# tjiiv-cprg/EPro-PnP

Hardware: AMD Instinct MI355X
Metric: PnP instances/sec (fwd+bwd, N=512 pts, 512 samples) (higher is better)
Workload: dtype f32; 1 GPU; C2 batched synthetic: 4096 objects/GPU x N=512 points, S=512 MC samples, K=4 AMIS iters, L=3 LM iters, EProPnP6DoF fwd+bwd; objects_per_gpu=4096, objects_total=4096, num_points=512, mc_samples=512, amis_iters=4, lm_iters=3, dof=6, parallelism=objects sharded x1, no data-path collective

## Files before the change

### epro-pnp_amd/csrc/amis_common.h

```cpp
#pragma once
#include "pnp_host.h"
#include "tuning.h"

namespace pnp {

typedef PNP_FIT_T fit_t;

__device__ __forceinline__ float sat_mul(float x, float one_v) {
  return __builtin_amdgcn_fmed3f(x * one_v, 0.0f, 1.0f);
}

__device__ __forceinline__ float sat_fma(float a, float b, float c) {
  return __builtin_amdgcn_fmed3f(fmaf(a, b, c), 0.0f, 1.0f);
}

__device__ __forceinline__ float clamp_below(float x, float lo) {
  int xi, li;
  memcpy(&xi, &x, 4);
  memcpy(&li, &lo, 4);
  const int mi = max(xi, li);
  float r;
  memcpy(&r, &mi, 4);
  return r;
}
// ... 8 lines not shown
  return h;
}

constexpr int kPropStride = 40;
constexpr int kVmTries = PNP_VM_TRIES;
constexpr int kRedStride = 68;
constexpr int kWaveRed = 16 * kRedStride + 64;

struct AmisParams {
  int S, K;
  int WP;
  float eps;
  int mle_iter;
  float dispersion;
  unsigned long long seed, offset;
  const unsigned long long* offset_dev;
  unsigned long long* advance;
  int* advance_ticket;
  int advance_count;
  int ablate;
  unsigned split_timeout;
  const float* dn_offset;
  float* dn_samples;
  float* dn_pose_opt;
  float* sample_costs;
};

template <int DOF>
PNP_FN void denormalise_pose_opt(const AmisParams& a, const float* __restrict__ pose_opt, int b) {
  constexpr int PL = PoseLen<DOF>::value;
  if (a.dn_offset == nullptr || a.dn_pose_opt == nullptr) return;
  float ps[PL], R[9];
#pragma unroll
  for (int i = 0; i < PL; ++i) ps[i] = pose_opt[(size_t)b * PL + i];
  pose_to_rot<DOF>(ps, R);
  shift_translation(ps, R, a.dn_offset[(size_t)b * 3], a.dn_offset[(size_t)b * 3 + 1], a.dn_offset[(size_t)b * 3 + 2], -1.0f);
#pragma unroll
  for (int i = 0; i < PL; ++i) a.dn_pose_opt[(size_t)b * PL + i] = ps[i];
}

__device__ __forceinline__ void advance_counters(const AmisParams& a, int expected) {
  if (a.advance == nullptr) return;
  if (threadIdx.x == 0) {
    if (atomicAdd(a.advance_ticket, 1) == expected - 1) {
      for (int i = 0; i < a.advance_count; ++i) atomicAdd(&a.advance[i], 1ull);
      atomicExch(a.advance_ticket, 0);
    }
  }
}


__device__ __forceinline__ constexpr int tri(int i, int j) { return i * (i + 1) / 2 + j; }


PNP_FIT_FN void fit_translation(fit_t (&C)[3][3], const float* fallback_diag, float* rec) {
  fit_t invd[3];
  const bool ok = cholesky<3, fit_t>(C, invd);
  rec[37] = ok ? 0.f : 1.f;
  if (!ok) {
#pragma unroll
    for (int i = 0; i < 3; ++i) {
#pragma unroll
      for (int j = 0; j < 3; ++j) C[i][j] = (i == j) ? (fit_t)fallback_diag[i] : fit_t(0);
      invd[i] = fit_t(1) / (fit_t)fallback_diag[i];
    }
  }
  fit_t Li[3][3];
  tri_inverse<3, fit_t>(C, invd, Li);
  float sl = 0.f;
#pragma unroll
  for (int i = 0; i < 3; ++i) {
    sl += fast_log((float)C[i][i]);
#pragma unroll
    for (int j = 0; j <= i; ++j) {
      rec[3 + tri(i, j)] = (float)C[i][j];
      rec[9 + tri(i, j)] = (float)Li[i][j];
    }
  }
  rec[15] = student_t3_log_norm(sl);
}

constexpr int kRefitMaxVals = 21;
constexpr int kRefitRedFloats = kRefitMaxVals * kSumTRow + 24;

template <int NV>
PNP_FN void wave_sum_t(float (&v)[NV], float* lds, int lane) {
  static_assert(NV <= kRefitMaxVals, "scratch rows");
  float* tot = lds + kRefitMaxVals * kSumTRow;
#pragma unroll
  for (int i = 0; i < NV; ++i) lds[i * kSumTRow + lane] = v[i];
  wave_lds_fence();
#pragma unroll
  for (int base = 0; base < NV; base += 16) {
    const int row = base + (lane >> 2);
    float part = 0.f;
    if (row < NV) {
      const float4* r = reinterpret_cast<const float4*>(lds + row * kSumTRow + 16 * (lane & 3));
      const float4 a = r[0], b = r[1], c = r[2], d = r[3];
      part = (((a.x + a.y) + (a.z + a.w)) + ((b.x + b.y) + (b.z + b.w))) + (((c.x + c.y) + (c.z + c.w)) + ((d.x + d.y) + (d.z + d.w)));
    }
    part = quad_sum(part);
    if (row < NV && (lane & 3) == 0) tot[row] = part;
  }
  wave_lds_fence();
#pragma unroll
  for (int i = 0; i < NV; ++i) v[i] = tot[i];
  wave_lds_fence();
}

template <int NV>
PNP_FN void refit_sum(float (&v)[NV], float* scratch, int lane) {
  if (scratch != nullptr) {
    wave_sum_t<NV>(v, scratch, lane);
  } else {
#pragma unroll
    for (int i = 0; i < NV; ++i) v[i] = wave_sum(v[i]);
  }
}

PNP_FIT_FN void fit_factor_pair(fit_t (&A)[4][4], int which, float dispersion, const float (&fallback)[4], float* rec) {
  const fit_t m01 = A[0][0] * A[1][1] - A[0][1] * A[1][0], m02 = A[0][0] * A[1][2] - A[0][2] * A[1][0],
               m03 = A[0][0] * A[1][3] - A[0][3] * A[1][0], m12 = A[0][1] * A[1][2] - A[0][2] * A[1][1],
               m13 = A[0][1] * A[1][3] - A[0][3] * A[1][1], m23 = A[0][2] * A[1][3] - A[0][3] * A[1][2];
  const fit_t n01 = A[2][0] * A[3][1] - A[2][1] * A[3][0], n02 = A[2][0] * A[3][2] - A[2][2] * A[3][0],
               n03 = A[2][0] * A[3][3] - A[2][3] * A[3][0], n12 = A[2][1] * A[3][2] - A[2][2] * A[3][1],
               n13 = A[2][1] * A[3][3] - A[2][3] * A[3][1], n23 = A[2][2] * A[3][3] - A[2][3] * A[3][2];
  const float det = (float)(m01 * n23 - m02 * n13 + m03 * n12 + m12 * n03 - m13 * n02 + m23 * n01);
  const fit_t add = (which == 0) ? (fit_t)(sqrtf(sqrtf(det)) * dispersion) : fit_t(0);
  fit_t invd[4];
#pragma unroll
  for (int i = 0; i < 4; ++i) A[i][i] += add;
  const bool ok = cholesky<4, fit_t>(A, invd) && (add == add);
  if (!ok) {
#pragma unroll
    for (int i = 0; i < 4; ++i) {
#pragma unroll
      for (int j = 0; j < 4; ++j) A[i][j] = (i == j) ? (fit_t)fallback[i] : fit_t(0);
      invd[i] = fit_t(1) / (fit_t)fallback[i];
    }
  }
  fit_t Li[4][4];
  tri_inverse<4, fit_t>(A, invd, Li);
  float sl = 0.f;
  const int oL = which ? 3 : 16, oLi = which ? 9 : 26;
#pragma unroll
  for (int i = 0; i < 4; ++i) {
    sl += fast_log((float)A[i][i]);
#pragma unroll
    for (int j = 0; j <= i; ++j) {
      if (which == 0 || i < 3) {
        rec[oL + tri(i, j)] = (float)A[i][j];
        rec[oLi + tri(i, j)] = (float)Li[i][j];
      }
    }
  }
  rec[which ? 15 : 36] = which ? student_t3_log_norm(sl) : sl;
  rec[which ? 37 : 38] = ok ? 0.f : 1.f;
}

template <int DOF>
PNP_FIT_FN void initial_fit(const float* pose_opt, const float* cov, float eps, float dispersion, float* rec, int which = 0) {
  if (which == 0) {
    rec[0] = pose_opt[0]; rec[1] = pose_opt[1]; rec[2] = pose_opt[2];
    rec[39] = 0.f;
  }
  if (DOF == 4) {
    rec[37] = rec[38] = 0.f;
    fit_t Ct[3][3];
#pragma unroll
    for (int i = 0; i < 3; ++i)
#pragma unroll
      for (int j = 0; j < 3; ++j) Ct[i][j] = (fit_t)cov[i * DOF + j];
    const float dflt[3] = {1.0f, 1.0f, 4.0f};
    fit_translation(Ct, dflt, rec);
    rec[16] = pose_opt[3];
    const float kappa = 0.33f / fmaxf(cov[3 * 4 + 3], eps);
    rec[17] = kappa;
    rec[18] = log_i0(kappa);
#pragma unroll
    for (int i = 19; i < 37; ++i) rec[i] = 0.f;
  } else {
    fit_t Cr[3][3], Ci[3][3];
#pragma unroll
    for (int i = 0; i < 3; ++i)
#pragma unroll
      for (int j = 0; j < 3; ++j) Cr[i][j] = (fit_t)cov[(3 + i) * 6 + 3 + j];
    fit_t invd4[4];
    {
      const fit_t c00 = Cr[1][1] * Cr[2][2] - Cr[1][2] * Cr[2][1], c01 = Cr[1][2] * Cr[2][0] - Cr[1][0] * Cr[2][2],
                   c02 = Cr[1][0] * Cr[2][1] - Cr[1][1] * Cr[2][0];
      const fit_t idet = fit_t(1) / (Cr[0][0] * c00 + Cr[0][1] * c01 + Cr[0][2] * c02);
      Ci[0][0] = c00 * idet; Ci[1][0] = c01 * idet; Ci[2][0] = c02 * idet;
      Ci[0][1] = (Cr[0][2] * Cr[2][1] - Cr[0][1] * Cr[2][2]) * idet;
      Ci[1][1] = (Cr[0][0] * Cr[2][2] - Cr[0][2] * Cr[2][0]) * idet;
      Ci[2][1] = (Cr[0][1] * Cr[2][0] - Cr[0][0] * Cr[2][1]) * idet;
      Ci[0][2] = (Cr[0][1] * Cr[1][2] - Cr[0][2] * Cr[1][1]) * idet;
// ... 249 lines not shown
        ps[3] = v0 * inr; ps[4] = v1 * inr; ps[5] = v2 * inr; ps[6] = v3 * inr;
      }
    } else {
      const int n_u = (int)rintf(0.25f * (float)s);
      auto uniforms = [&](int att, float& u1, float& u2, float& u3) {
        if (noise != nullptr) {
          const float* nz = noise + (((size_t)b * K + it) * s + n) * NZ + 4 + 3 * att;
          u1 = nz[0]; u2 = nz[1]; u3 = nz[2];
        } else {
          const Philox4 r = philox4x32_10((uint32_t)b, (uint32_t)m, (uint32_t)a.offset,
                                          (uint32_t)(a.offset >> 32) * 64u + 8u + (uint32_t)att, (uint32_t)a.seed,
                                          (uint32_t)(a.seed >> 32));
          u1 = (float)(r.v[0] >> 8) * (1.0f / 16777216.0f);
          u2 = (float)(r.v[1] >> 8) * (1.0f / 16777216.0f);
          u3 = (float)(r.v[2] >> 8) * (1.0f / 16777216.0f);
        }
      };
      if (n < n_u) {
        float u1, u2, u3;
        uniforms(0, u1, u2, u3);
        ps[3] = (u1 * 2.0f - 1.0f) * 3.14159265358979f;
      } else {
        ps[3] = vm_sample_bounded(rec[16], rec[17], uniforms);
      }
    }
    PNP_REFIT_ADD(3, rot_t0_);
#pragma unroll
    for (int i = 0; i < PL; ++i) smp[i * S + m] = ps[i];
    if (pose_samples != nullptr) store_pose<PL>(pose_samples + ((size_t)m * p.B + b) * PL, ps);
    {
      float R[9], KR[9], Kt[3];
      pose_to_rot<DOF>(ps, R);
      if (pose_samples != nullptr && a.dn_samples != nullptr) {
        float pd[PL];
#pragma unroll
        for (int i = 0; i < PL; ++i) pd[i] = ps[i];
        shift_translation(pd, R, a.dn_offset[(size_t)b * 3], a.dn_offset[(size_t)b * 3 + 1], a.dn_offset[(size_t)b * 3 + 2], -1.0f);
        store_pose<PL>(a.dn_samples + ((size_t)m * p.B + b) * PL, pd);
      }
      compose_kr_kt(Kc, R, ps, KR, Kt);
      float4* row = reinterpret_cast<float4*>(ptab + 12 * (n - n0));
      row[0] = make_float4(KR[0], KR[1], KR[2], Kt[0]);
      row[1] = make_float4(KR[3], KR[4], KR[5], Kt[1]);
      row[2] = make_float4(KR[6], KR[7], KR[8], Kt[2]);
    }
  }

}

template <int DOF>
PNP_FN void amis_weights(const AmisCtx& cx, const AmisParams& a, int it, int WP) {
  constexpr int PL = PoseLen<DOF>::value;
  float* smp = cx.smp; float* cst = cx.cst; float* mixl = cx.mixl; float* lgw = cx.lgw; float* cpart = cx.cpart; float* prop = cx.prop;
  const int S = cx.S, s = cx.s, T = cx.T, tid = cx.tid;
  const float* rec = prop + it * kPropStride;
  const int M = (it + 1) * s;
  const float log_n = logf((float)(it + 1));
  for (int m = tid; m < M; m += T) {
    float ps[PL];
#pragma unroll
    for (int i = 0; i < PL; ++i) ps[i] = smp[i * S + m];
    float mix;
    if (m >= it * s) {
      if (WP > 0) {
        float c = cpart[m - it * s];
        for (int q = 1; q < WP; ++q) c += cpart[q * cx.cstride + (m - it * s)];
        cst[m] = c;
      }
      if (PNP_ABLATED(a, 4)) {
        mix = 0.f;
      } else {
        mix = proposal_logprob<DOF>(prop, ps);
        for (int j = 1; j <= it; ++j) mix = log_add_exp(mix, proposal_logprob<DOF>(prop + j * kPropStride, ps));
      }
    } else {
      mix = PNP_ABLATED(a, 4) ? 0.f : log_add_exp(mixl[m], proposal_logprob<DOF>(rec, ps));
    }
    mixl[m] = mix;
    lgw[m] = -cst[m] - (mix - log_n);
  }

}

template <int DOF>
PNP_FN void amis_refit(const AmisCtx& cx, const AmisParams& a, int it) {
  float* smp = cx.smp; float* lgw = cx.lgw; float* prop = cx.prop; float* red = cx.red;
  const int S = cx.S, s = cx.s;
  const float* rec = prop + it * kPropStride;
  const int M = (it + 1) * s;
  float* nrec = prop + (it + 1) * kPropStride;
  if (wave_id() != 0) {
    amis_base_noise<DOF>(cx, a, it + 1, 64);
    __syncthreads();
    return;
  }
  const int T = 64, tid = cx.tid;
  PNP_REFIT_BEGIN();
  if (PNP_ABLATED(a, 2)) {
    for (int i = tid; i < kPropStride; i += T) nrec[i] = rec[i];
    __syncthreads();
    return;
  }
  float mx = -INFINITY;
  for (int m = tid; m < M; m += T) mx = fmaxf(mx, lgw[m]);
  mx = wave_max(mx);
  const float p0 = rec[0], p1 = rec[1], p2 = rec[2];
  if (DOF == 6) {
    float mom[21];
#pragma unroll
    for (int i = 0; i < 21; ++i) mom[i] = 0.f;
    if (PNP_ABLATED(a, 8)) mom[0] = mom[4] = mom[6] = mom[9] = mom[10] = mom[12] = mom[15] = mom[19] = mom[20] = 1.f;
    else
    for (int m = tid; m < M; m += T) {
      const float e = fast_exp(lgw[m] - mx);
      const float d0 = smp[m] - p0, d1 = smp[S + m] - p1, d2 = smp[2 * S + m] - p2;
      mom[0] += e;
      mom[1] += e * d0; mom[2] += e * d1; mom[3] += e * d2;
      mom[4] += e * d0 * d0; mom[5] += e * d1 * d0; mom[6] += e * d1 * d1;
      mom[7] += e * d2 * d0; mom[8] += e * d2 * d1; mom[9] += e * d2 * d2;
      const float q0 = smp[3 * S + m], q1 = smp[4 * S + m], q2 = smp[5 * S + m], q3 = smp[6 * S + m];
      const float iw = e * fast_rcp(fmaxf(q0 * q0 + q1 * q1 + q2 * q2 + q3 * q3, a.eps));
      mom[10] += iw * q0 * q0;
      mom[11] += iw * q1 * q0; mom[12] += iw * q1 * q1;
      mom[13] += iw * q2 * q0; mom[14] += iw * q2 * q1; mom[15] += iw * q2 * q2;
      mom[16] += iw * q3 * q0; mom[17] += iw * q3 * q1; mom[18] += iw * q3 * q2; mom[19] += iw * q3 * q3;
      mom[20] += iw;
    }
    if (!PNP_ABLATED(a, 16)) refit_sum<21>(mom, cx.rred, tid);
    const float invZ = 1.0f / mom[0];
    const float dl0 = mom[1] * invZ, dl1 = mom[2] * invZ, dl2 = mom[3] * invZ;
    const float mu0 = p0 + dl0, mu1 = p1 + dl1, mu2 = p2 + dl2;
    float c6[6];
    c6[0] = mom[4] * invZ - dl0 * dl0; c6[1] = mom[5] * invZ - dl1 * dl0; c6[2] = mom[6] * invZ - dl1 * dl1;
    c6[3] = mom[7] * invZ - dl2 * dl0; c6[4] = mom[8] * invZ - dl2 * dl1; c6[5] = mom[9] * invZ - dl2 * dl2;
    float acc[11];
#pragma unroll
    for (int i = 0; i < 11; ++i) acc[i] = mom[10 + i];
    PNP_REFIT_PHASE(0);
    float Lf[10], Ld[4];
    for (int r = 1; r < a.mle_iter; ++r) {
      if (tid == 0) {
        fit_t Sg[4][4], invd[4];
        const fit_t inorm = fit_t(1) / (fit_t)acc[10];
#pragma unroll
        for (int i = 0; i < 4; ++i)
#pragma unroll
          for (int j = 0; j <= i; ++j) {
            const fit_t v = (fit_t)acc[tri(i, j)] * inorm + ((i == j) ? (fit_t)a.eps : fit_t(0));
            Sg[i][j] = v;
            Sg[j][i] = v;
          }
        cholesky<4, fit_t>(Sg, invd);
#pragma unroll
        for (int i = 0; i < 4; ++i) {
          red[10 + i] = (float)invd[i];
#pragma unroll
          for (int j = 0; j < i; ++j) red[tri(i, j)] = (float)Sg[i][j];
        }
      }
      wave_lds_fence();
#pragma unroll
      for (int i = 0; i < 10; ++i) Lf[i] = red[i];
#pragma unroll
      for (int i = 0; i < 4; ++i) Ld[i] = red[10 + i];
      wave_lds_fence();
#pragma unroll
      for (int i = 0; i < 11; ++i) acc[i] = 0.f;
      for (int m = tid; m < M; m += T) {
        const float e = fast_exp(lgw[m] - mx);
        const float q0 = smp[3 * S + m], q1 = smp[4 * S + m], q2 = smp[5 * S + m], q3 = smp[6 * S + m];
        const float y0 = q0 * Ld[0];
        const float y1 = fmaf(-Lf[tri(1, 0)], y0, q1) * Ld[1];
        const float y2 = fmaf(-Lf[tri(2, 1)], y1, fmaf(-Lf[tri(2, 0)], y0, q2)) * Ld[2];
        const float y3 = fmaf(-Lf[tri(3, 2)], y2, fmaf(-Lf[tri(3, 1)], y1, fmaf(-Lf[tri(3, 0)], y0, q3))) * Ld[3];
        const float Mq = fmaf(y3, y3, fmaf(y2, y2, fmaf(y1, y1, y0 * y0)));
        const float iw = e * fast_rcp(fmaxf(Mq, a.eps));
        acc[10] += iw;
        acc[0] += iw * q0 * q0;
        acc[1] += iw * q1 * q0; acc[2] += iw * q1 * q1;
        acc[3] += iw * q2 * q0; acc[4] += iw * q2 * q1; acc[5] += iw * q2 * q2;
        acc[6] += iw * q3 * q0; acc[7] += iw * q3 * q1; acc[8] += iw * q3 * q2; acc[9] += iw * q3 * q3;
      }
      refit_sum<11>(acc, cx.rred, tid);
    }
    PNP_REFIT_PHASE(1);
    if (tid < 2) {
      if (tid == 0) {
        nrec[0] = mu0; nrec[1] = mu1; nrec[2] = mu2;
        nrec[39] = 0.f;
      }
      fit_t A4[4][4];
      const fit_t inorm = (a.mle_iter > 0) ? fit_t(1) / (fit_t)acc[10] : fit_t(0);
#pragma unroll
      for (int i = 0; i < 4; ++i)
#pragma unroll
        for (int j = 0; j <= i; ++j) {
          fit_t v = (a.mle_iter > 0) ? (fit_t)acc[tri(i, j)] * inorm + ((i == j) ? (fit_t)a.eps : fit_t(0))
                                      : ((i == j) ? fit_t(1) : fit_t(0));
          if (tid == 1) v = (i < 3) ? (fit_t)c6[tri(i, j)] : ((i == j) ? fit_t(1) : fit_t(0));
          A4[i][j] = v;
          A4[j][i] = v;
        }
      const float dflt[4] = {1.f, 1.f, 1.f, 1.f};
      fit_factor_pair(A4, tid, a.dispersion, dflt, nrec);
    }
    PNP_REFIT_PHASE(2);
  } else {
    float mom[12];
#pragma unroll
    for (int i = 0; i < 12; ++i) mom[i] = 0.f;
    for (int m = tid; m < M; m += T) {
      const float e = fast_exp(lgw[m] - mx);
      const float d0 = smp[m] - p0, d1 = smp[S + m] - p1, d2 = smp[2 * S + m] - p2;
      mom[0] += e;
      mom[1] += e * d0; mom[2] += e * d1; mom[3] += e * d2;
      mom[4] += e * d0 * d0; mom[5] += e * d1 * d0; mom[6] += e * d1 * d1;
      mom[7] += e * d2 * d0; mom[8] += e * d2 * d1; mom[9] += e * d2 * d2;
      const float yaw = smp[3 * S + m];
      float sy, cy;
      sincos_rad(yaw, sy, cy);
      mom[10] += e * sy;
      mom[11] += e * cy;
    }
    refit_sum<12>(mom, cx.rred, tid);
    const float invZ = 1.0f / mom[0];
    const float dl0 = mom[1] * invZ, dl1 = mom[2] * invZ, dl2 = mom[3] * invZ;
    const float mu0 = p0 + dl0, mu1 = p1 + dl1, mu2 = p2 + dl2;
    float c8[8];
    c8[0] = mom[4] * invZ - dl0 * dl0; c8[1] = mom[5] * invZ - dl1 * dl0; c8[2] = mom[6] * invZ - dl1 * dl1;
    c8[3] = mom[7] * invZ - dl2 * dl0; c8[4] = mom[8] * invZ - dl2 * dl1; c8[5] = mom[9] * invZ - dl2 * dl2;
    c8[6] = mom[10] * invZ;
    c8[7] = mom[11] * invZ;
    if (tid == 0) {
      nrec[0] = mu0; nrec[1] = mu1; nrec[2] = mu2;
      fit_t Ct[3][3];
#pragma unroll
      for (int i = 0; i < 3; ++i)
#pragma unroll
        for (int j = 0; j <= i; ++j) {
          Ct[i][j] = (fit_t)c8[tri(i, j)];
          Ct[j][i] = (fit_t)c8[tri(i, j)];
        }
      const float dflt[3] = {1.f, 1.f, 4.f};
      nrec[38] = nrec[39] = 0.f;
      fit_translation(Ct, dflt, nrec);
      nrec[16] = atan2f(c8[6], c8[7]);
      const float r_sq = c8[6] * c8[6] + c8[7] * c8[7];
      const float kappa = 0.33f * fmaxf(sqrtf(r_sq), a.eps) * (2.f - r_sq) / fmaxf(1.f - r_sq, a.eps);
      nrec[17] = kappa;
      nrec[18] = log_i0(kappa);
#pragma unroll
      for (int i = 19; i < 37; ++i) nrec[i] = 0.f;
    }
  }
  __syncthreads();
}

}
```

### epro-pnp_amd/csrc/amis_forward_mfma.hip

```cpp
#include "amis_common.h"
#include "dispatch.h"

namespace pnp {



template <bool BOUNDS, bool FOLDED = false>
__device__ __forceinline__ void huber_cost_4(const floatx4& hx, const floatx4& hy, const floatx4& hz, const float4& w4,
                                             float zmin_v, float one_v, const Bounds& bd, f32x2 (&acc2)[2]) {
  static_assert(!(BOUNDS && FOLDED), "the clamp acts on the un-weighted projection");
  const f32x2 wu2 = {w4.x, w4.x}, wv2 = {w4.y, w4.y}, cu2 = {w4.z, w4.z}, cv2 = {w4.w, w4.w};
  const f32x2 mhalf = {-0.5f, -0.5f};
#pragma unroll
  for (int h = 0; h < 2; ++h) {
    const float z0 = clamp_below(hz[2 * h], zmin_v), z1 = clamp_below(hz[2 * h + 1], zmin_v);
    const f32x2 rz2 = {fast_rcp(z0), fast_rcp(z1)};
    const f32x2 hx2 = {hx[2 * h], hx[2 * h + 1]}, hy2 = {hy[2 * h], hy[2 * h + 1]};
    f32x2 rx2, ry2;
    if (FOLDED) {
      rx2 = fma2(hx2, rz2, cu2);
      ry2 = fma2(hy2, rz2, cv2);
    } else {
      f32x2 px2 = hx2 * rz2, py2 = hy2 * rz2;
      if (BOUNDS) {
        px2 = f32x2{clamp_lu(px2[0], bd.lbx, bd.ubx), clamp_lu(px2[1], bd.lbx, bd.ubx)};
        py2 = f32x2{clamp_lu(py2[0], bd.lby, bd.uby), clamp_lu(py2[1], bd.lby, bd.uby)};
      }
      rx2 = fma2(px2, wu2, cu2);
      ry2 = fma2(py2, wv2, cv2);
    }
    const f32x2 s2 = fma2(rx2, rx2, ry2 * ry2);
    const f32x2 rho2 = {fast_sqrt(s2[0]), fast_sqrt(s2[1])};
    const f32x2 m2 = {sat_mul(rho2[0], one_v), sat_mul(rho2[1], one_v)};
    acc2[h] = fma2(m2, fma2(mhalf, m2, rho2), acc2[h]);
  }
}

constexpr int kChunk = 1024;

struct MfmaShape {
  int chunk;
  int s16;
  int ahead;
  int chunks;
};

template <int DOF, bool BOUNDS, int NPT, bool SPILL = false, bool SPLIT = false, bool BF16 = false, bool CHUNKED = false>
__global__ __launch_bounds__(512, SPLIT ? 2 : (DOF == 6 ? (NPT <= 8 ? (BF16 ? PNP_FWD_BF16_MINW : PNP_FWD_MINW) : 2) : (NPT <= 2 ? 3 : 2))) void amis_forward_mfma_kernel(Problem p, AmisParams a_in, MfmaShape sh,
                                                                  const float* __restrict__ pose_opt,
                                                                  const float* __restrict__ pose_cov,
                                                                  const float* __restrict__ noise,
                                                                  float* __restrict__ pose_samples,
                                                                  float* __restrict__ logweights,
                                                                  float* __restrict__ proposals,
                                                                  float* __restrict__ spill, int nsplit,
                                                                  float* __restrict__ xch) {
  static_assert(!SPILL || NPT == 0, "the spill variant streams the points");
  static_assert(!SPLIT || NPT > 0, "the split over workgroups is a register-mode variant");
  constexpr int PL = PoseLen<DOF>::value;
  const int G = SPLIT ? nsplit : 1;
  static_assert(!CHUNKED || (NPT > 0 && !SPLIT && !SPILL), "chunks are a register-mode variant of the one-workgroup kernel");
  const int CH = CHUNKED ? sh.chunks : 1;
  const int GT = SPLIT ? G : CH;
  int b, part = 0;
  if (SPLIT) {
    const int g = (int)blockIdx.x, per = (p.B + 7) >> 3, idx = g >> 3;
    part = idx % G;
    b = (g & 7) * per + idx / G;
  } else {
    b = object_of_block(p.B);
  }
  if (b >= p.B) return;
  AmisParams a = a_in;
  if (a.offset_dev != nullptr) a.offset += *a.offset_dev;
  const int T = (int)blockDim.x, tid = (int)threadIdx.x, lane = lane_id(), wv = wave_id(), W = T >> 6;
  const int S = a.S, K = a.K, s = S / K, s16 = sh.s16, NC = sh.chunk;

  PNP_PHASES_BEGIN(6);
  PNP_DYN_SMEM(float, smem);
  constexpr bool kRegs = NPT > 0;
  static_assert(!BF16 || NPT > 0, "the split projection is a register-mode variant");
  constexpr bool kBf = BF16;
  typedef ProjOp<kBf> Proj;
  constexpr bool kFold = kRegs && !BOUNDS && !kBf;
  const int WPs = kRegs ? (G > 1 ? G : W) : 1;
  const int cpart_rows = kRegs ? (SPLIT ? W + G : W) : 1;
  float* ptab = smem;
  float* pB = ptab + 12 * s16;
  float* pW = pB + 4 * NC;
  float* smp = SPILL ? spill + (size_t)b * (PL + 3) * S : pW + 4 * NC;
  float* cst = smp + PL * S;
  float* mixl = cst + S;
  float* lgw = mixl + S;
  float* cpart = SPILL ? pW + 4 * NC : smp + (((PL + 3) * S + 3) & ~3);
  float* gath = cpart + W * s16;
  float* prop = cpart + cpart_rows * s16 + (SPLIT ? 4 : 0);
  float* red = prop + K * kPropStride;
  float* rred = red + 256;
  float* nzb = (s <= T) ? ptab : rred + kRefitRedFloats;

  float Kc[9], delta;
  Bounds bd;
  load_camera<BOUNDS>(p, b, Kc, bd, delta);
  const float zmin_v = to_vgpr(p.z_min), one_v = to_vgpr(1.0f);
  const HuberScale hs = huber_scale(delta);
  const float inv_delta = hs.inv_delta, delta_sq = hs.delta_sq;

  const bool tiled = SPILL && s > s16;
  AmisCtx cx;
  cx.ptab = ptab; cx.smp = smp; cx.cst = cst; cx.mixl = mixl; cx.lgw = lgw; cx.cpart = SPLIT ? gath : cpart; cx.prop = prop; cx.red = red;
  cx.S = S; cx.K = K; cx.s = s; cx.T = T; cx.tid = tid; cx.b = b; cx.cstride = s16;
  cx.nzb = (noise == nullptr && W > 1 && sh.ahead) ? nzb : nullptr;
  cx.rred = rred;

  if (!tiled)
    for (int i = tid; i < 12 * (s16 - s); i += T) ptab[12 * s + i] = 0.f;
  if (tid < (DOF == 6 ? 2 : 1))
    initial_fit<DOF>(pose_opt + (size_t)b * PL, pose_cov + (size_t)b * DOF * DOF, a.eps, a.dispersion, prop, tid);
  if (part == 0 && tid == T - 1) denormalise_pose_opt<DOF>(a, pose_opt, b);
  const int nchunk = kRegs ? 1 : (p.N + NC - 1) / NC;
  auto load_chunk = [&](int c0) {
    const int cnt = min(NC, ((p.N - c0 + 15) >> 4) << 4);
    for (int n = tid; n < cnt; n += T) {
      const Point q = load_point(p, b, c0 + n);
      reinterpret_cast<float4*>(pB)[n] = make_float4(q.X, q.Y, q.Z, 1.0f);
      const float wu = q.wu * inv_delta, wv = q.wv * inv_delta;
      reinterpret_cast<float4*>(pW)[n] = make_float4(wu, wv, -q.u * wu, -q.v * wv);
    }
  };
  typename Proj::T rB[kRegs ? NPT : 1];
  float4 rW[kRegs ? NPT : 1];
  auto load_tiles = [&](int pt) {
#pragma unroll
    for (int i = 0; i < (kRegs ? NPT : 1); ++i) {
      const Point q = load_point(p, b, ((pt * W + wv) + GT * W * i) * 16 + (lane & 15));
      const int k4 = lane >> 4;
      const float bval = (k4 == 0) ? q.X : (k4 == 1) ? q.Y : (k4 == 2) ? q.Z : 1.0f;
      rB[i] = Proj::b(bval);
      const float wu = q.wu * inv_delta, wv = q.wv * inv_delta;
      rW[i] = kFold ? make_float4(bval * wu, bval * wv, -q.u * wu, -q.v * wv) : make_float4(wu, wv, -q.u * wu, -q.v * wv);
    }
  };
  if (kRegs) {
    if constexpr (!CHUNKED) load_tiles(part);
  } else if (nchunk == 1) {
    load_chunk(0);
  }
  amis_base_noise<DOF>(cx, a, 0, 64);
  __syncthreads();

  const int g4 = (lane >> 4) * 4, col = lane & 15, kk = lane >> 4;
  auto sweep_regs = [&](bool accumulate = false) {
    const floatx4 zero = {0.f, 0.f, 0.f, 0.f};
    for (int t = 0; t < (s16 >> 4); ++t) {
      const float* arow = ptab + 12 * (t * 16 + col) + kk;
      const typename Proj::T ax = Proj::a(arow[0]), ay = Proj::a(arow[4]), az = Proj::a(arow[8]);
      f32x2 acc2[2] = {f32x2{0.f, 0.f}, f32x2{0.f, 0.f}};
      constexpr int NT = kRegs ? NPT : 1;
      constexpr bool kPipe = (PNP_FWD_PIPE != 0) && !kFold && NT >= 4;
      floatx4 hxn = zero, hyn = zero, hzn = zero;
      if (kPipe) {
        hxn = Proj::mma(ax, rB[0], zero); hyn = Proj::mma(ay, rB[0], zero); hzn = Proj::mma(az, rB[0], zero);
      }
#pragma unroll
      for (int i = 0; i < NT; ++i) {
        floatx4 hx, hy, hz;
        if constexpr (kFold) {
          hx = mfma_16x16x4(ax, rW[i].x, zero);
          hy = mfma_16x16x4(ay, rW[i].y, zero);
          hz = mfma_16x16x4(az, rB[i], zero);
        } else if constexpr (kPipe) {
          hx = hxn; hy = hyn; hz = hzn;
          if (i + 1 < NT) {
            hxn = Proj::mma(ax, rB[i + 1], zero);
            hyn = Proj::mma(ay, rB[i + 1], zero);
            hzn = Proj::mma(az, rB[i + 1], zero);
            sched_fence();
          }
        } else {
          hx = Proj::mma(ax, rB[i], zero);
          hy = Proj::mma(ay, rB[i], zero);
          hz = Proj::mma(az, rB[i], zero);
        }
        huber_cost_4<BOUNDS, kFold>(hx, hy, hz, rW[i], zmin_v, one_v, bd, acc2);
      }
      const float acc[4] = {acc2[0][0], acc2[0][1], acc2[1][0], acc2[1][1]};
      const float tot = row_sum16_of4(acc);
      if (col < 4) {
        float* dst = cpart + wv * s16 + t * 16 + g4 + col;
        if constexpr (CHUNKED) *dst = accumulate ? fmaf(tot, delta_sq, *dst) : tot * delta_sq;
        else *dst = tot * delta_sq;
      }
    }
  };
  PNP_PHASE(0);
  unsigned gone_parts = 0u;
  for (int it = 0; it < K; ++it) {
    for (int n0 = 0; n0 < (SPILL ? s : 1); n0 += (SPILL ? s16 : 1)) {
    const int cnt = min(s16, s - n0), cnt16 = (cnt + 15) & ~15;
    if (tiled) {
      if (n0 > 0) __syncthreads();
      for (int i = tid; i < 12 * (cnt16 - cnt); i += T) ptab[12 * cnt + i] = 0.f;
    }
    if (!PNP_ABLATED(a, 32) || it == 0)
      amis_draw<DOF>(cx, p, a, it, Kc, noise, part == 0 ? pose_samples : nullptr, n0, tiled ? cnt : -1);
    __syncthreads();
    PNP_PHASE(1);

    if (PNP_ABLATED(a, 1)) {
      for (int n = tid; n < s; n += T) cpart[n] = 1.0f;
    } else if (kRegs) {
      if constexpr (!CHUNKED) {
        sweep_regs();
      } else {
        for (int c = 0; c < CH; ++c) {
          load_tiles(c);
          sweep_regs(c > 0);
        }
      }
    } else
    for (int ch = 0; ch < nchunk; ++ch) {
      const int c0 = ch * NC;
      if (nchunk > 1) {
        if (ch > 0 || it > 0) __syncthreads();
        load_chunk(c0);
        __syncthreads();
      }
      const int npt = (min(NC, p.N - c0) + 15) >> 4;
      for (int t = wv; t < (cnt16 >> 4); t += W) {
        const float* arow = ptab + 12 * (t * 16 + col) + kk;
        const float ax = arow[0], ay = arow[4], az = arow[8];
        f32x2 acc2[2] = {f32x2{0.f, 0.f}, f32x2{0.f, 0.f}};
        const floatx4 zero = {0.f, 0.f, 0.f, 0.f};
        float bq = pB[4 * col + kk];
        float4 w4 = reinterpret_cast<const float4*>(pW)[col];
        floatx4 hx = mfma_16x16x4(ax, bq, zero), hy = mfma_16x16x4(ay, bq, zero), hz = mfma_16x16x4(az, bq, zero);
        for (int q = 0; q < npt; ++q) {
          const int qn = min(q + 1, npt - 1);
          const float bn = pB[4 * (qn * 16 + col) + kk];
          const float4 wn = reinterpret_cast<const float4*>(pW)[qn * 16 + col];
          const floatx4 hxn = mfma_16x16x4(ax, bn, zero);
          const floatx4 hyn = mfma_16x16x4(ay, bn, zero);
          const floatx4 hzn = mfma_16x16x4(az, bn, zero);
          huber_cost_4<BOUNDS>(hx, hy, hz, w4, zmin_v, one_v, bd, acc2);
          hx = hxn; hy = hyn; hz = hzn; w4 = wn;
        }
        const float acc[4] = {acc2[0][0], acc2[0][1], acc2[1][0], acc2[1][1]};
        const float tot = row_sum16_of4(acc);
        if (col < 4) {
          const int pose = t * 16 + g4 + col;
          cpart[pose] = (ch == 0) ? tot * delta_sq : fmaf(tot, delta_sq, cpart[pose]);
        }
      }
    }
    __syncthreads();
    if (tiled)
      for (int m = tid; m < cnt; m += T) cst[it * s + n0 + m] = cpart[m];
    }
    if (kRegs && SPLIT) {
      unsigned* slot = reinterpret_cast<unsigned*>(xch) + (((size_t)b * K + it) * G) * s16;
      unsigned* missw = reinterpret_cast<unsigned*>(gath + G * s16);
      for (int m = tid; m < s; m += T) {
        float c = cpart[m];
        for (int w = 1; w < W; ++w) c += cpart[w * s16 + m];
        const unsigned bits = xwg_payload(c);
        xwg_store(slot + part * s16 + m, bits);
        gath[part * s16 + m] = bits_f32(bits);
      }
      if (tid == 0) *missw = 0u;
      __syncthreads();
      unsigned miss = 0u;
      for (int i = tid; i < G * s; i += T) {
        const int q = i / s, m = i - q * s;
        if (q == part) continue;
        const unsigned v = xwg_poll(slot + q * s16 + m, (((miss | gone_parts) >> q) & 1u) ? 0u : a.split_timeout);
        if (v == kXwgEmpty) miss |= 1u << q; else gath[q * s16 + m] = bits_f32(v);
      }
      if (miss) atomicOr(reinterpret_cast<int*>(missw), (int)miss);
      __syncthreads();
      unsigned todo = *missw;
      gone_parts |= todo;
      if (todo) {
        if (tid == 0) raise_status(p, EPROPNP_ST_SPLIT_TIMEOUT, b);
        for (int q = 0; q < G; ++q) {
          if (!((todo >> q) & 1u)) continue;
          load_tiles(q);
          sweep_regs();
          __syncthreads();
          for (int m = tid; m < s; m += T) {
            float c = cpart[m];
            for (int w = 1; w < W; ++w) c += cpart[w * s16 + m];
            gath[q * s16 + m] = bits_f32(xwg_payload(c));
          }
          __syncthreads();
        }
        load_tiles(part);
      }
    }
    PNP_PHASE(2);

    if (tiled) __syncthreads();
    AmisCtx cxw = cx;
    cxw.tid = (int)f32_bits(to_vgpr(bits_f32((unsigned)tid)));
    amis_weights<DOF>(cxw, a, it, tiled ? 0 : WPs);
    __syncthreads();
    PNP_PHASE(3);
    if (it == K - 1) break;
    amis_refit<DOF>(cxw, a, it);
    PNP_PHASE(4);
  }

  if (part == 0) {
    int st_bits = 0;
    for (int m = tid; m < S; m += T) {
      const float lw = lgw[m];
      logweights[(size_t)m * p.B + b] = lw;
      if (a.sample_costs != nullptr) a.sample_costs[(size_t)m * p.B + b] = cst[m];
      st_bits |= (lw == lw && lw != INFINITY) ? 0 : EPROPNP_ST_NONFINITE_WEIGHT;
    }
    for (int i = tid; i < K; i += T)
      st_bits |= (prop[i * kPropStride + 37] != 0.f || prop[i * kPropStride + 38] != 0.f) ? EPROPNP_ST_CHOL_FALLBACK : 0;
    raise_status(p, st_bits, b);
  }
  if (proposals != nullptr && part == 0)
    for (int i = tid; i < K * kPropStride; i += T) proposals[(size_t)b * K * kPropStride + i] = prop[i];
  PNP_PHASE(5);
  advance_counters(a, p.B * G);
  PNP_PHASES_FLUSH(6);
}

int tuning_phase_cycles(unsigned long long* out, int reset) { return tuning::read_cycles(out, reset, true); }

template <class F>
static int dispatch_npt(int npt, F&& f) {
  switch (npt) {
    case 0: return f(ic<0>{});
    case 1: return f(ic<1>{});
    case 2: return f(ic<2>{});
    case 4: return f(ic<4>{});
    case 8: return f(ic<8>{});
    case 12: return f(ic<12>{});
    default: return f(ic<16>{});
  }
}

static int forward_split_parts(int B, int ptiles) {
  const long wgs = padded_object_grid(B), cus = device_cu_count();
  int g = 8;
  while (g > 1 && (wgs * g > cus || 8 * g > ptiles)) g >>= 1;
  if (g < 4) g = 1;
  { int ov[1]; if (env_ints("EPROPNP_FWD_SPLIT", ov, 1) && (ov[0] == 1 || ov[0] == 2 || ov[0] == 4 || ov[0] == 8) && wgs * ov[0] <= 4096 && 4 * ov[0] <= ptiles) g = ov[0]; }
  return g;
}

unsigned long long amis_forward_split_bytes(const epropnp_problem* prob, int mc_samples, int num_iter) {
  if (prob == nullptr || prob->num_obj <= 0 || num_iter <= 0 || mc_samples % num_iter != 0) return 0;
  const int ptiles = (prob->num_pts + 15) / 16;
  const int g = forward_split_parts(prob->num_obj, ptiles);
  if (g <= 1 || (ptiles + 4 * g - 1) / (4 * g) > 8) return 0;
  const int s16 = ((mc_samples / num_iter + 15) / 16) * 16;
  return sizeof(float) * (unsigned long long)prob->num_obj * num_iter * g * s16;
}

struct FwdPlan {
  MfmaShape sh;
  int waves, npt, G;
  size_t smem;
  bool bf16, spilled, truncated, chunked;
};

static int plan_amis_forward(const epropnp_problem* prob, int S, int K, unsigned long long scratch_bytes, FwdPlan* out) {
  const int B = prob->num_obj, N = prob->num_pts;
  const int s = S / K;
  const int PL = prob->dof == 6 ? 7 : 4;
  MfmaShape& sh = out->sh;
  sh.s16 = ((s + 15) / 16) * 16;
  const int ptiles = (N + 15) / 16;
  const int npt_opts[6] = {1, 2, 4, 8, 12, 16};
  int waves = 4, npt = 0, best = 1 << 30;
  for (int w : {4, 8, 2, 1}) {
    for (int o : npt_opts) {
      if (w * o >= ptiles && w * o < best) { best = w * o; waves = w; npt = o; }
      if (w * o >= ptiles) break;
    }
  }
  if (prob->dof == 4 && npt >= 12) npt = 0;
  if (B < 512 && waves == 4 && npt == 8) { waves = 8; npt = 4; }
  { int ov[2]; if (tune_ints("fwd_mfma", ov, 2) && (ov[0] == 1 || ov[0] == 2 || ov[0] == 4 || ov[0] == 8) && (ov[1] == 0 || ov[1] == 1 || ov[1] == 2 || ov[1] == 4 || ov[1] == 8 || ov[1] == 12 || ov[1] == 16) && (ov[1] == 0 || ov[0] * ov[1] >= ptiles)) { waves = ov[0]; npt = ov[1]; } }
  if (npt == 0) {
    sh.chunk = ((N + 15) / 16) * 16;
    if (sh.chunk > kChunk) sh.chunk = kChunk;
    if (best == (1 << 30)) waves = 4;
    const int tiles = sh.s16 / 16;
    while (waves > 1 && waves > tiles) waves /= 2;
  } else {
    sh.chunk = 0;
  }
  int G = 1;
  {
    const int g = forward_split_parts(B, ptiles);
    const size_t need = sizeof(float) * (size_t)B * K * g * sh.s16;
    int ovf[1];
    const bool forced = env_ints("EPROPNP_FWD_SPLIT", ovf, 1);
    if (g > 1 && (forced || (scratch_bytes != 0 && scratch_bytes >= need))) {
      int per_wave = (ptiles + 4 * g - 1) / (4 * g), o = 1;
      while (o < per_wave) o *= 2;
      if (o <= 8) { G = g; waves = 4; npt = o; sh.chunk = 0; }
    }
  }
  sh.chunks = 1;
  { const char* e = getenv("EPROPNP_FWD_PROJ"); if (e && e[0] == 'f') sh.chunks = 0; }
  if (sh.chunks == 1 && G == 1 && npt > 8 && ptiles > 48 && !tune_flag("fwd_no_chunks") && !tune_flag("fwd_mfma")) {
    waves = 4; npt = 8;
    sh.chunks = (ptiles + 31) / 32;
  }
  if (sh.chunks < 1) sh.chunks = 1;
  sh.ahead = 1;
  auto lds_bytes = [&](bool spilled) {
    return sizeof(float) * (12 * (size_t)sh.s16 + 8 * (size_t)sh.chunk + (spilled ? 0 : (((size_t)(PL + 3) * S + 3) & ~(size_t)3)) +
                            (size_t)(npt ? (G > 1 ? waves + G : waves) : 1) * sh.s16 + (G > 1 ? 4 : 0) + (size_t)K * kPropStride + 256 +
                            kRefitRedFloats +
                            ((s <= 64 * waves || !sh.ahead) ? 0 : 8 * (size_t)s));
  };
  size_t smem = lds_bytes(false);
  const int s16_full = sh.s16;
  bool spilled = false;
  if (smem > 160 * 1024) {
    spilled = true;
    waves = 8; npt = 0; G = 1; sh.chunks = 1;
    sh.chunk = ((N + 15) / 16) * 16;
    if (sh.chunk > kChunk) sh.chunk = kChunk;
    const int tiles = sh.s16 / 16;
    while (waves > 1 && waves > tiles) waves /= 2;
    smem = lds_bytes(true);
    if (smem > 160 * 1024) {
      sh.ahead = 0;
      const size_t fixed = sizeof(float) * (8 * (size_t)sh.chunk + (size_t)K * kPropStride + 256 + kRefitRedFloats);
      const size_t rows = (160 * 1024 - fixed) / (sizeof(float) * 13);
      if ((size_t)sh.s16 > rows) sh.s16 = (int)(rows / 16) * 16;
      if (sh.s16 < 16) return fail(EPROPNP_EINVAL, "amis_forward: no LDS left for a pose tile (%d points per chunk)", sh.chunk);
      smem = lds_bytes(true);
    }
  }
  bool bf16 = npt >= 1;
  if (const char* e = getenv("EPROPNP_FWD_PROJ")) bf16 = (e[0] == 'f') ? false : bf16;
  out->waves = waves; out->npt = npt; out->G = G; out->smem = smem;
  out->bf16 = bf16; out->spilled = spilled; out->truncated = sh.s16 < s16_full;
  out->chunked = !spilled && G == 1 && npt == 8 && (sh.chunks > 1 || (bf16 && tune_flag("fwd_chunked")));
  return EPROPNP_OK;
}

int plan_amis_forward_record(const epropnp_problem* prob, int S, int K, unsigned long long scratch_bytes, int32_t* out) {
  FwdPlan plan;
  if (int rc = plan_amis_forward(prob, S, K, scratch_bytes, &plan)) return rc;
  out[0] = plan.waves; out[1] = plan.npt; out[2] = plan.G; out[3] = plan.sh.chunks; out[4] = plan.bf16; out[5] = plan.spilled;
  out[6] = plan.truncated; out[7] = plan.chunked;
  return EPROPNP_OK;
}

int launch_amis_forward_mfma(const epropnp_problem* prob, const epropnp_amis_params* am, const float* pose_opt,
                             const float* pose_cov, const float* noise, float* pose_samples, float* logweights,
                             float* proposals, hipStream_t st, const DenormOut* dn, float* sample_costs) {
  const Problem d = to_device_problem(prob);
  const int S = am->mc_samples, K = am->num_iter;
  const int PL = prob->dof == 6 ? 7 : 4;
  FwdPlan plan;
  if (int rc = plan_amis_forward(prob, S, K, am->split_scratch != nullptr ? am->split_scratch_bytes : 0, &plan)) return rc;
  const MfmaShape sh = plan.sh;
  const int waves = plan.waves, npt = plan.npt, G = plan.G;
  const size_t smem = plan.smem;
  const bool bf16 = plan.bf16;
  AmisParams k;
  k.S = S; k.K = K; k.WP = 1; k.eps = am->eps; k.mle_iter = am->acg_mle_iter; k.dispersion = am->acg_dispersion;
  k.seed = am->seed; k.offset = am->offset; k.offset_dev = (const unsigned long long*)am->offset_dev; k.ablate = 0;
  k.advance = (am->advance && am->advance_ticket && am->advance_count > 0) ? (unsigned long long*)am->advance : nullptr;
  k.advance_ticket = (int*)am->advance_ticket; k.advance_count = am->advance_count;
  k.split_timeout = split_timeout_cycles();
  k.dn_offset = dn ? dn->offset : nullptr; k.dn_samples = dn ? dn->samples : nullptr; k.dn_pose_opt = dn ? dn->pose_opt : nullptr;
  k.sample_costs = sample_costs;
  { int ab[1]; if (tune_ints("ablate", ab, 1)) k.ablate = ab[0]; }
  float* spill = nullptr;
  if (plan.spilled &&
      hipMallocAsync((void**)&spill, sizeof(float) * (size_t)(PL + 3) * S * d.B, st) != hipSuccess) {
    (void)hipGetLastError();
    return fail(EPROPNP_ELAUNCH, "amis_forward: mc_samples %d needs a %zu B scratch buffer and hipMallocAsync failed "
                "(stream capture?)", S, sizeof(float) * (size_t)(PL + 3) * S * d.B);
  }
  const dim3 grid(padded_object_grid(d.B)), block(64 * waves);
  if (spill != nullptr) {
    dispatch_dof_bounds(prob->dof, has_bounds(prob), [&](auto DOF, auto BND) -> int {
      auto kern = amis_forward_mfma_kernel<decltype(DOF)::value, decltype(BND)::value, 0, true>;
      allow_dynamic_lds((const void*)kern, smem);
      PNP_LAUNCH(kern, grid, block, smem, st, d, k, sh, pose_opt, pose_cov, noise, pose_samples, logweights, proposals, spill, 1,
                 (float*)nullptr);
      return 0;
    });
    const int rc = check_launch("amis_forward_mfma_kernel (sampler state in global scratch)");
    (void)hipFreeAsync(spill, st);
    return rc;
  }
  float* xch = nullptr;
  char* owned = nullptr;
  dim3 grid_split = grid;
  if (G > 1) {
    const size_t xbytes = sizeof(float) * (size_t)d.B * K * G * sh.s16;
    char* mem = (am->split_scratch != nullptr && am->split_scratch_bytes >= xbytes) ? (char*)am->split_scratch : nullptr;
    if (mem == nullptr) {
      if (hipMallocAsync((void**)&mem, xbytes, st) != hipSuccess) {
        (void)hipGetLastError();
        return fail(EPROPNP_ELAUNCH, "amis_forward: scratch for the %d-way split (%zu B) could not be allocated", G, xbytes);
      }
      owned = mem;
    }
    if (!exchange_prefilled(mem, xbytes) &&
        launch_fill_u32(mem, 0xffffffffu, xbytes / 4, st) != EPROPNP_OK) {
      (void)hipGetLastError();
      return fail(EPROPNP_ELAUNCH, "amis_forward: could not fill the split scratch");
    }
    xch = (float*)mem;
    grid_split = dim3(padded_object_grid(d.B) * G);
  }
  if (G > 1) {
    dispatch_dof_bounds(prob->dof, has_bounds(prob), [&](auto DOF, auto BND) -> int {
      auto go = [&](auto NPT) -> int {
        auto run = [&](auto kern) -> int {
          allow_dynamic_lds((const void*)kern, smem);
          PNP_LAUNCH(kern, grid_split, block, smem, st, d, k, sh, pose_opt, pose_cov, noise, pose_samples, logweights, proposals,
                     (float*)nullptr, G, xch);
          return 0;
        };
        if (bf16) return run(amis_forward_mfma_kernel<decltype(DOF)::value, decltype(BND)::value, decltype(NPT)::value, false, true, true>);
        return run(amis_forward_mfma_kernel<decltype(DOF)::value, decltype(BND)::value, decltype(NPT)::value, false, true>);
      };
      switch (npt) {
        case 1: return go(ic<1>{});
        case 2: return go(ic<2>{});
        case 4: return go(ic<4>{});
        default: return go(ic<8>{});
      }
    });
  } else {
    dispatch_dof_bounds(prob->dof, has_bounds(prob), [&](auto DOF, auto BND) -> int {
      return dispatch_npt(npt, [&](auto NPT) -> int {
        auto run = [&](auto kern) -> int {
          allow_dynamic_lds((const void*)kern, smem);
          PNP_LAUNCH(kern, grid, block, smem, st, d, k, sh, pose_opt, pose_cov, noise, pose_samples, logweights, proposals,
                     (float*)nullptr, 1, (float*)nullptr);
          return 0;
        };
        if constexpr (decltype(NPT)::value == 8) {
          if (plan.chunked)
            return run(amis_forward_mfma_kernel<decltype(DOF)::value, decltype(BND)::value, 8, false, false, true, true>);
        }
        if constexpr (decltype(NPT)::value >= 1) {
          if (bf16) return run(amis_forward_mfma_kernel<decltype(DOF)::value, decltype(BND)::value, decltype(NPT)::value, false, false, true>);
        }
        return run(amis_forward_mfma_kernel<decltype(DOF)::value, decltype(BND)::value, decltype(NPT)::value>);
      });
    });
  }
  if (owned != nullptr) (void)hipFreeAsync(owned, st);
  return check_launch("amis_forward_mfma_kernel");
}

}
```

### epro-pnp_amd/csrc/tuning.h

```cpp
#pragma once

#ifndef PNP_FIT_T
#define PNP_FIT_T double
#endif
#ifndef PNP_FIT_FN
#define PNP_FIT_FN __device__ __forceinline__
#endif
#ifndef PNP_VM_TRIES
#define PNP_VM_TRIES 16
#endif
#ifndef PNP_FWD_BF16_MINW
#define PNP_FWD_BF16_MINW 3
#endif
#ifndef PNP_FWD_PIPE
#define PNP_FWD_PIPE 1
#endif
#ifndef PNP_FWD_MINW
#define PNP_FWD_MINW 4
#endif
#ifndef PNP_BWD_MINW4
#define PNP_BWD_MINW4 2
#endif
#ifndef PNP_BWD_MINW
#define PNP_BWD_MINW 3
#endif

#ifdef PNP_TUNING
#define PNP_ABLATED(par, bit) ((((par).ablate) & (bit)) != 0)
#define PNP_PHASES_BEGIN(n)                \
  long long phase_t0_ = clock64();         \
  unsigned long long phase_acc_[n] = {}
#define PNP_PHASE(i)                                                   \
  do {                                                                 \
    if (tid == 0) {                                                    \
      const long long now_ = clock64();                                \
      phase_acc_[i] += (unsigned long long)(now_ - phase_t0_);         \
      phase_t0_ = now_;                                                \
    }                                                                  \
  } while (0)
#define PNP_PHASES_FLUSH(n)                                                                      \
  do {                                                                                           \
    if (tid == 0) {                                                                              \
      for (int i_ = 0; i_ < (n); ++i_) atomicAdd(&::pnp::tuning::g_phase[i_], phase_acc_[i_]);   \
    }                                                                                            \
  } while (0)
#else
#define PNP_ABLATED(par, bit) false
#define PNP_PHASES_BEGIN(n)
#define PNP_PHASE(i)
#define PNP_PHASES_FLUSH(n)
#endif

#if defined(PNP_TUNING) && defined(PNP_TUNING_REFIT)
#define PNP_REFIT_BEGIN() long long refit_t0_ = clock64()
#define PNP_REFIT_PHASE(i)                                                                      \
  do {                                                                                          \
    if (tid == 0) {                                                                             \
      const long long now_ = clock64();                                                         \
      atomicAdd(&::pnp::tuning::g_refit_phase[i], (unsigned long long)(now_ - refit_t0_));      \
      refit_t0_ = now_;                                                                         \
    }                                                                                           \
  } while (0)
#define PNP_REFIT_CLOCK(name) const long long name = clock64()
#define PNP_REFIT_ADD(i, name)                                                                                      \
  do {                                                                                                              \
    if (tid == 0) atomicAdd(&::pnp::tuning::g_refit_phase[i], (unsigned long long)(clock64() - (name)));            \
  } while (0)
#else
#define PNP_REFIT_BEGIN()
#define PNP_REFIT_PHASE(i)
#define PNP_REFIT_CLOCK(name)
#define PNP_REFIT_ADD(i, name)
#endif

namespace pnp {
namespace tuning {
#ifdef PNP_TUNING
static __device__ unsigned long long g_phase[8];
static __device__ unsigned long long g_refit_phase[4];
static inline int read_cycles(unsigned long long* out, int reset, bool with_refit) {
  if (out && hipMemcpyFromSymbol(out, HIP_SYMBOL(g_phase), sizeof(unsigned long long) * 8) != hipSuccess) return -1;
  if (with_refit && out) {
    unsigned long long rf[4];
    if (hipMemcpyFromSymbol(rf, HIP_SYMBOL(g_refit_phase), sizeof(rf)) != hipSuccess) return -1;
    out[6] = rf[1];
    out[7] = rf[2];
  }
  if (reset) {
    const unsigned long long z[8] = {0, 0, 0, 0, 0, 0, 0, 0};
    if (hipMemcpyToSymbol(HIP_SYMBOL(g_phase), z, sizeof(z)) != hipSuccess) return -1;
    if (hipMemcpyToSymbol(HIP_SYMBOL(g_refit_phase), z, sizeof(unsigned long long) * 4) != hipSuccess) return -1;
  }
  return 0;
}
#else
// ... 5 lines not shown
```

Measured before the change: 3.023 million instances/s.

## Move per-point Huber weights to LDS to raise forward kernel occupancy

Adds a WLDS variant of the bf16 6-DoF one-workgroup forward kernel. It stores the per-point weight float4s in LDS instead of registers and prefetches them one step ahead in the cost loop. This frees VGPRs so launch bounds can ask for 4 workgroups per CU instead of 3. To keep LDS within budget, the refit reduction scratch is cut to 11 rows and aliased onto the cpart buffer, and the 21 moments are reduced in two halves. The trade is extra LDS traffic, an extra reduction pass and aliasing risk, in return for higher occupancy. The variant is chosen by the planner only when 4 workgroups fit in the per-CU LDS and the grid is large enough.

```diff
diff --git a/epro-pnp_amd/csrc/amis_common.h b/epro-pnp_amd/csrc/amis_common.h
--- a/epro-pnp_amd/csrc/amis_common.h
+++ b/epro-pnp_amd/csrc/amis_common.h
@@ -114,11 +114,13 @@
 
 constexpr int kRefitMaxVals = 21;
 constexpr int kRefitRedFloats = kRefitMaxVals * kSumTRow + 24;
-
-template <int NV>
+constexpr int kRefitHalfVals = 11;
+constexpr int kRefitHalfFloats = kRefitHalfVals * kSumTRow + 24;
+
+template <int NV, int ROWS = kRefitMaxVals>
 PNP_FN void wave_sum_t(float (&v)[NV], float* lds, int lane) {
-  static_assert(NV <= kRefitMaxVals, "scratch rows");
-  float* tot = lds + kRefitMaxVals * kSumTRow;
+  static_assert(NV <= ROWS, "scratch rows");
+  float* tot = lds + ROWS * kSumTRow;
 #pragma unroll
   for (int i = 0; i < NV; ++i) lds[i * kSumTRow + lane] = v[i];
   wave_lds_fence();
@@ -140,10 +142,10 @@
   wave_lds_fence();
 }
 
-template <int NV>
+template <int NV, int ROWS = kRefitMaxVals>
 PNP_FN void refit_sum(float (&v)[NV], float* scratch, int lane) {
   if (scratch != nullptr) {
-    wave_sum_t<NV>(v, scratch, lane);
+    wave_sum_t<NV, ROWS>(v, scratch, lane);
   } else {
 #pragma unroll
     for (int i = 0; i < NV; ++i) v[i] = wave_sum(v[i]);
@@ -559,8 +561,10 @@
 
 }
 
-template <int DOF>
+template <int DOF, bool HALF = false>
 PNP_FN void amis_refit(const AmisCtx& cx, const AmisParams& a, int it) {
+  static_assert(!HALF || DOF == 6, "the half-size scratch serves the 6-DoF refit");
+  constexpr int ROWS = HALF ? kRefitHalfVals : kRefitMaxVals;
   float* smp = cx.smp; float* lgw = cx.lgw; float* prop = cx.prop; float* red = cx.red;
   const int S = cx.S, s = cx.s;
   const float* rec = prop + it * kPropStride;
@@ -603,7 +607,23 @@
       mom[16] += iw * q3 * q0; mom[17] += iw * q3 * q1; mom[18] += iw * q3 * q2; mom[19] += iw * q3 * q3;
       mom[20] += iw;
     }
-    if (!PNP_ABLATED(a, 16)) refit_sum<21>(mom, cx.rred, tid);
+    if (!PNP_ABLATED(a, 16)) {
+      if constexpr (HALF) {
+        float lo[11], hi[10];
+#pragma unroll
+        for (int i = 0; i < 11; ++i) lo[i] = mom[i];
+#pragma unroll
+        for (int i = 0; i < 10; ++i) hi[i] = mom[11 + i];
+        refit_sum<11, ROWS>(lo, cx.rred, tid);
+        refit_sum<10, ROWS>(hi, cx.rred, tid);
+#pragma unroll
+        for (int i = 0; i < 11; ++i) mom[i] = lo[i];
+#pragma unroll
+        for (int i = 0; i < 10; ++i) mom[11 + i] = hi[i];
+      } else {
+        refit_sum<21>(mom, cx.rred, tid);
+      }
+    }
     const float invZ = 1.0f / mom[0];
     const float dl0 = mom[1] * invZ, dl1 = mom[2] * invZ, dl2 = mom[3] * invZ;
     const float mu0 = p0 + dl0, mu1 = p1 + dl1, mu2 = p2 + dl2;
@@ -658,7 +678,7 @@
         acc[3] += iw * q2 * q0; acc[4] += iw * q2 * q1; acc[5] += iw * q2 * q2;
         acc[6] += iw * q3 * q0; acc[7] += iw * q3 * q1; acc[8] += iw * q3 * q2; acc[9] += iw * q3 * q3;
       }
-      refit_sum<11>(acc, cx.rred, tid);
+      refit_sum<11, ROWS>(acc, cx.rred, tid);
     }
     PNP_REFIT_PHASE(1);
     if (tid < 2) {
diff --git a/epro-pnp_amd/csrc/amis_forward_mfma.hip b/epro-pnp_amd/csrc/amis_forward_mfma.hip
--- a/epro-pnp_amd/csrc/amis_forward_mfma.hip
+++ b/epro-pnp_amd/csrc/amis_forward_mfma.hip
@@ -45,8 +45,8 @@
   int chunks;
 };
 
-template <int DOF, bool BOUNDS, int NPT, bool SPILL = false, bool SPLIT = false, bool BF16 = false, bool CHUNKED = false>
-__global__ __launch_bounds__(512, SPLIT ? 2 : (DOF == 6 ? (NPT <= 8 ? (BF16 ? PNP_FWD_BF16_MINW : PNP_FWD_MINW) : 2) : (NPT <= 2 ? 3 : 2))) void amis_forward_mfma_kernel(Problem p, AmisParams a_in, MfmaShape sh,
+template <int DOF, bool BOUNDS, int NPT, bool SPILL = false, bool SPLIT = false, bool BF16 = false, bool CHUNKED = false, bool WLDS = false>
+__global__ __launch_bounds__(512, SPLIT ? 2 : (DOF == 6 ? (NPT <= 8 ? (BF16 ? (WLDS ? PNP_FWD_WLDS_MINW : PNP_FWD_BF16_MINW) : PNP_FWD_MINW) : 2) : (NPT <= 2 ? 3 : 2))) void amis_forward_mfma_kernel(Problem p, AmisParams a_in, MfmaShape sh,
                                                                   const float* __restrict__ pose_opt,
                                                                   const float* __restrict__ pose_cov,
                                                                   const float* __restrict__ noise,
@@ -57,6 +57,7 @@
                                                                   float* __restrict__ xch) {
   static_assert(!SPILL || NPT == 0, "the spill variant streams the points");
   static_assert(!SPLIT || NPT > 0, "the split over workgroups is a register-mode variant");
+  static_assert(!WLDS || (BF16 && DOF == 6 && NPT > 0 && !SPLIT && !CHUNKED && !SPILL), "weights in LDS: the one-workgroup bf16 6-DoF kernel");
   constexpr int PL = PoseLen<DOF>::value;
   const int G = SPLIT ? nsplit : 1;
   static_assert(!CHUNKED || (NPT > 0 && !SPLIT && !SPILL), "chunks are a register-mode variant of the one-workgroup kernel");
@@ -94,10 +95,11 @@
   float* lgw = mixl + S;
   float* cpart = SPILL ? pW + 4 * NC : smp + (((PL + 3) * S + 3) & ~3);
   float* gath = cpart + W * s16;
-  float* prop = cpart + cpart_rows * s16 + (SPLIT ? 4 : 0);
+  float* prop = cpart + (WLDS ? max(cpart_rows * s16, kRefitHalfFloats) : cpart_rows * s16) + (SPLIT ? 4 : 0);
   float* red = prop + K * kPropStride;
-  float* rred = red + 256;
-  float* nzb = (s <= T) ? ptab : rred + kRefitRedFloats;
+  float* wl = red + 256;
+  float* rred = WLDS ? cpart : red + 256;
+  float* nzb = (s <= T) ? ptab : (WLDS ? wl + W * NPT * 64 : rred + kRefitRedFloats);
 
   float Kc[9], delta;
   Bounds bd;
@@ -135,10 +137,15 @@
     for (int i = 0; i < (kRegs ? NPT : 1); ++i) {
       const Point q = load_point(p, b, ((pt * W + wv) + GT * W * i) * 16 + (lane & 15));
       const int k4 = lane >> 4;
+      const int wslot = (wv * NPT + i) * 16 + (lane & 15);
       const float bval = (k4 == 0) ? q.X : (k4 == 1) ? q.Y : (k4 == 2) ? q.Z : 1.0f;
       rB[i] = Proj::b(bval);
       const float wu = q.wu * inv_delta, wv = q.wv * inv_delta;
-      rW[i] = kFold ? make_float4(bval * wu, bval * wv, -q.u * wu, -q.v * wv) : make_float4(wu, wv, -q.u * wu, -q.v * wv);
+      if constexpr (WLDS) {
+        if (k4 == 0) reinterpret_cast<float4*>(wl)[wslot] = make_float4(wu, wv, -q.u * wu, -q.v * wv);
+      } else {
+        rW[i] = kFold ? make_float4(bval * wu, bval * wv, -q.u * wu, -q.v * wv) : make_float4(wu, wv, -q.u * wu, -q.v * wv);
+      }
     }
   };
   if (kRegs) {
@@ -159,12 +166,20 @@
       constexpr int NT = kRegs ? NPT : 1;
       constexpr bool kPipe = (PNP_FWD_PIPE != 0) && !kFold && NT >= 4;
       floatx4 hxn = zero, hyn = zero, hzn = zero;
+      const float4* wl4 = reinterpret_cast<const float4*>(wl) + wv * NPT * 16 + col;
+      float4 wn = make_float4(0.f, 0.f, 0.f, 0.f);
+      if constexpr (WLDS) wn = wl4[0];
       if (kPipe) {
         hxn = Proj::mma(ax, rB[0], zero); hyn = Proj::mma(ay, rB[0], zero); hzn = Proj::mma(az, rB[0], zero);
       }
 #pragma unroll
       for (int i = 0; i < NT; ++i) {
         floatx4 hx, hy, hz;
+        float4 w4 = rW[i];
+        if constexpr (WLDS) {
+          w4 = wn;
+          if (!kPipe && i + 1 < NT) wn = wl4[16 * (i + 1)];
+        }
         if constexpr (kFold) {
           hx = mfma_16x16x4(ax, rW[i].x, zero);
           hy = mfma_16x16x4(ay, rW[i].y, zero);
@@ -172,6 +187,7 @@
         } else if constexpr (kPipe) {
           hx = hxn; hy = hyn; hz = hzn;
           if (i + 1 < NT) {
+            if constexpr (WLDS) wn = wl4[16 * (i + 1)];
             hxn = Proj::mma(ax, rB[i + 1], zero);
             hyn = Proj::mma(ay, rB[i + 1], zero);
             hzn = Proj::mma(az, rB[i + 1], zero);
@@ -182,7 +198,7 @@
           hy = Proj::mma(ay, rB[i], zero);
           hz = Proj::mma(az, rB[i], zero);
         }
-        huber_cost_4<BOUNDS, kFold>(hx, hy, hz, rW[i], zmin_v, one_v, bd, acc2);
+        huber_cost_4<BOUNDS, kFold>(hx, hy, hz, w4, zmin_v, one_v, bd, acc2);
       }
       const float acc[4] = {acc2[0][0], acc2[0][1], acc2[1][0], acc2[1][1]};
       const float tot = row_sum16_of4(acc);
@@ -306,7 +322,7 @@
     __syncthreads();
     PNP_PHASE(3);
     if (it == K - 1) break;
-    amis_refit<DOF>(cxw, a, it);
+    amis_refit<DOF, WLDS>(cxw, a, it);
     PNP_PHASE(4);
   }
 
@@ -367,7 +383,10 @@
   int waves, npt, G;
   size_t smem;
   bool bf16, spilled, truncated, chunked;
+  bool wlds;
 };
+
+constexpr size_t kLdsPerCu = 160 * 1024, kLdsGranule = 1280;
 
 static int plan_amis_forward(const epropnp_problem* prob, int S, int K, unsigned long long scratch_bytes, FwdPlan* out) {
   const int B = prob->num_obj, N = prob->num_pts;
@@ -416,10 +435,12 @@
   }
   if (sh.chunks < 1) sh.chunks = 1;
   sh.ahead = 1;
-  auto lds_bytes = [&](bool spilled) {
+  auto lds_bytes = [&](bool spilled, bool wlds = false) {
+    size_t cp = (size_t)(npt ? (G > 1 ? waves + G : waves) : 1) * sh.s16;
+    if (wlds && cp < (size_t)kRefitHalfFloats) cp = kRefitHalfFloats;
     return sizeof(float) * (12 * (size_t)sh.s16 + 8 * (size_t)sh.chunk + (spilled ? 0 : (((size_t)(PL + 3) * S + 3) & ~(size_t)3)) +
-                            (size_t)(npt ? (G > 1 ? waves + G : waves) : 1) * sh.s16 + (G > 1 ? 4 : 0) + (size_t)K * kPropStride + 256 +
-                            kRefitRedFloats +
+                            cp + (G > 1 ? 4 : 0) + (size_t)K * kPropStride + 256 +
+                            (wlds ? (size_t)64 * waves * npt : (size_t)kRefitRedFloats) +
                             ((s <= 64 * waves || !sh.ahead) ? 0 : 8 * (size_t)s));
   };
   size_t smem = lds_bytes(false);
@@ -447,6 +468,18 @@
   out->waves = waves; out->npt = npt; out->G = G; out->smem = smem;
   out->bf16 = bf16; out->spilled = spilled; out->truncated = sh.s16 < s16_full;
   out->chunked = !spilled && G == 1 && npt == 8 && (sh.chunks > 1 || (bf16 && tune_flag("fwd_chunked")));
+  out->wlds = false;
+  if (prob->dof == 6 && bf16 && !spilled && !out->chunked && G == 1 && waves == 4 && npt == 8) {
+    const size_t smem_w = lds_bytes(false, true);
+    const size_t granules = (smem_w + kLdsGranule - 1) / kLdsGranule * kLdsGranule;
+    bool take = 4 * granules <= kLdsPerCu && (long)padded_object_grid(B) > 3L * device_cu_count();
+    { int ov[1]; if (tune_ints("fwd_wlds", ov, 1)) take = ov[0] != 0 && smem_w <= kLdsPerCu; }
+    if (take) { out->wlds = true; out->smem = smem_w; }
+    if (take && PNP_FWD_WLDS_MINW < 4) {
+      const size_t hold = kLdsPerCu / PNP_FWD_WLDS_MINW / kLdsGranule * kLdsGranule;
+      if (out->smem < hold) out->smem = hold;
+    }
+  }
   return EPROPNP_OK;
 }
 
@@ -551,6 +584,10 @@
         if constexpr (decltype(NPT)::value == 8) {
           if (plan.chunked)
             return run(amis_forward_mfma_kernel<decltype(DOF)::value, decltype(BND)::value, 8, false, false, true, true>);
+          if constexpr (decltype(DOF)::value == 6) {
+            if (plan.wlds)
+              return run(amis_forward_mfma_kernel<6, decltype(BND)::value, 8, false, false, true, false, true>);
+          }
         }
         if constexpr (decltype(NPT)::value >= 1) {
           if (bf16) return run(amis_forward_mfma_kernel<decltype(DOF)::value, decltype(BND)::value, decltype(NPT)::value, false, false, true>);
diff --git a/epro-pnp_amd/csrc/tuning.h b/epro-pnp_amd/csrc/tuning.h
--- a/epro-pnp_amd/csrc/tuning.h
+++ b/epro-pnp_amd/csrc/tuning.h
@@ -11,6 +11,9 @@
 #endif
 #ifndef PNP_FWD_BF16_MINW
 #define PNP_FWD_BF16_MINW 3
+#endif
+#ifndef PNP_FWD_WLDS_MINW
+#define PNP_FWD_WLDS_MINW 4
 #endif
 #ifndef PNP_FWD_PIPE
 #define PNP_FWD_PIPE 1
```

Result: faster. 3.066 million instances/s (median of 6 runs) (+1.4%).
